# Gallicchio-Lab/openmm_agbnp_plugin

Measured on AMD Instinct MI355X. Metric: AGBNP1 force-eval-limited ns/day (1 fs step), thrombin 1dwc, independent replicas, higher is better.
Workload: dtype f64

## Files before the change

openmm_agbnp_plugin_amd/csrc/decompose_kernels.hip:

```cpp
#define AGBNP_GROUP_TU
#include "pair_bodies.h"

namespace agbnp {

__device__ __forceinline__ void decompose_atoms(const PairArgs& P, int version, int i, double* __restrict__ per_atom) {
  if (i >= P.n) return;
  const size_t n = (size_t)P.n;
  const int h = P.a2h[i];
  if (h >= 0) hbm_add(&per_atom[i], P.gam_cav[h] * (P.sv_large[h] - P.sv_vdw[h]));
  if (version != 1) return;
  const double b = P.born[i], q = P.charge[i], bh = b + kHBRadius;
  hbm_add(&per_atom[n + i], P.alpha[i] / (bh * bh * bh));
  hbm_add(&per_atom[2 * n + i], kDielFactor * q * q / b);
}

template <bool kCut>
__device__ __forceinline__ void decompose_tile(const PairArgs& P, int tile, double* __restrict__ plane) {
  __shared__ double2 s_xy[128], s_zq[128], s_bb[128];
  __shared__ double2 s_ixy[64], s_izq[64], s_ibc[64];
  __shared__ double s_red[4][2][64];
  __shared__ double s_box[2][6];
  const int n = P.n, nb = (n + 63) >> 6;
  if (tile >= nb * (nb + 1) / 2) return;
  int I = (int)(0.5 * ((double)(2 * nb + 1) - sqrt((double)(2 * nb + 1) * (double)(2 * nb + 1) - 8.0 * (double)tile)));
  I = max(0, min(I, nb - 1));
  while (I > 0 && I * nb - I * (I - 1) / 2 > tile) I--;
  while (I + 1 < nb && (I + 1) * nb - (I + 1) * I / 2 <= tile) I++;
  const int J = I + (tile - (I * nb - I * (I - 1) / 2));
  const int lane = threadIdx.x & 63, wave = threadIdx.x >> 6;
  const bool diag = I == J;
  if (wave < 2) {
    const int a = 64 * (wave == 0 ? J : I) + lane;
    const bool va = a < n;
    const int ac = va ? a : n - 1;
    const double4 pa = P.aposq[ac];
    const double br = P.born[ac], inv_br = 1.0 / br;
    const double qa = va ? pa.w : 0.0;
    if (wave == 0) {
      s_xy[lane] = s_xy[lane + 64] = make_double2(pa.x, pa.y);
      s_zq[lane] = s_zq[lane + 64] = make_double2(pa.z, qa);
      s_bb[lane] = s_bb[lane + 64] = make_double2(br, inv_br);
    } else {
      s_ixy[lane] = make_double2(pa.x, pa.y);
      s_izq[lane] = make_double2(pa.z, qa);
      s_ibc[lane] = make_double2(br, (-0.25 * 1.4426950408889634074) * inv_br);
    }
    if (kCut && !diag) {
      double lo[3] = {pa.x, pa.y, pa.z}, hi[3] = {pa.x, pa.y, pa.z};
      for (int off = 32; off > 0; off >>= 1)
        for (int d = 0; d < 3; d++) {
          lo[d] = fmin(lo[d], __shfl_xor(lo[d], off, 64));
          hi[d] = fmax(hi[d], __shfl_xor(hi[d], off, 64));
        }
      if (lane == 0)
        for (int d = 0; d < 3; d++) s_box[wave][d] = lo[d], s_box[wave][3 + d] = hi[d];
    }
  }
  __syncthreads();
  if (kCut && !diag) {
    if (box_gap2(&s_box[0][0], 0, 1) >= P.gb_cut2) return;
  }
  const int nsteps = diag ? 8 : 16;
  const int start = (diag ? 1 : 0) + nsteps * wave;
  const double2 ixy = s_ixy[lane], izq = s_izq[lane], ibc = s_ibc[lane];
  const double xi = ixy.x, yi = ixy.y, zi = izq.x, qi = izq.y, bi = ibc.x, ci = ibc.y;
  const int masked_step = diag ? 32 - start : -1;
  const double qlast = lane >= 32 ? 0.0 : qi;
  const int base = (lane + start) & 63;
  const double2* __restrict__ jxy = s_xy + base;
  const double2* __restrict__ jzq = s_zq + base;
  const double2* __restrict__ jbb = s_bb + base;
  double ei = 0.0, ej = 0.0;
#pragma unroll 8
  for (int k = 0; k < nsteps; k++) {
    const double2 xy = jxy[k], zq = jzq[k], bj = jbb[k];
    const double dx = xy.x - xi, dy = xy.y - yi, dz = zq.x - zi;
    const double d2 = fma(dz, dz, fma(dy, dy, dx * dx));
    double qq = (k == masked_step ? qlast : qi) * zq.y;
// ... 40 lines not shown
```

openmm_agbnp_plugin_amd/csrc/device_math.h:

```cpp
#pragma once
#include <hip/hip_runtime.h>

namespace agbnp {

__device__ __forceinline__ double exp2_nonpositive(double y) {
  y = fmax(y, -96.0);
  const double kShift = 6755399441055744.0;
  const double t = y + kShift;
  const double f = y - (t - kShift);
  double p = 0x1.e6063f7217bc6p-28;
  p = fma(p, f, 0x1.b675bca4eeebbp-24);
  p = fma(p, f, 0x1.62bfd47773353p-20);
  p = fma(p, f, 0x1.ffcb54062e698p-17);
  p = fma(p, f, 0x1.430913096fd9fp-13);
  p = fma(p, f, 0x1.5d87fe9d7a584p-10);
  p = fma(p, f, 0x1.3b2ab6fba1ddap-7);
  p = fma(p, f, 0x1.c6b08d703ce49p-5);
  p = fma(p, f, 0x1.ebfbdff82c598p-3);
  p = fma(p, f, 0x1.62e42fefa3a19p-1);
  p = fma(p, f, 1.0);
  const int n = __double2loint(t);
  return __hiloint2double(__double2hiint(p) + (n << 20), __double2loint(p));
}

__device__ __forceinline__ double rsqrt_pos(double u) {
  const double y0 = __builtin_amdgcn_rsq(u);
  const double e = fma(-(u * y0), y0, 1.0);
  return fma(y0 * e, fma(0.375, e, 0.5), y0);
}

__device__ __forceinline__ double exp_nonpositive(double x) { return exp2_nonpositive(x * 1.4426950408889634074); }

constexpr double kQGrad = 17179869184.0;
constexpr double kQVol = 4503599627370496.0;
constexpr double kQBorn = 17592186044416.0;
constexpr double kQSum = 1099511627776.0;
constexpr double kQEnergy = 68719476736.0;
__device__ __forceinline__ double quantize(double v, double scale, bool det) { return det ? rint(v * scale) * (1.0 / scale) : v; }

__device__ __forceinline__ double pow_three_halves(double q) { return (q * q) * rsqrt_pos(q); }

}
```

openmm_agbnp_plugin_amd/csrc/pair_bodies.h:

```cpp
#pragma once
#include <hip/hip_runtime.h>

#include <algorithm>

#include "agbnp_common.h"
#include "device_math.h"
#include "pair_kernels.h"
#include "group_args.h"
#include "prep_role.h"

namespace agbnp {

#ifdef AGBNP_PAIR_STAMPS
constexpr int kPairLogSlots = 4096;
__device__ unsigned long long g_pair_log[3][kPairLogSlots][12];
#define PAIR_STAMP(kern, idx)                                                                                        \
  do {                                                                                                               \
    if (threadIdx.x == 0 && blockIdx.x < kPairLogSlots) g_pair_log[kern][blockIdx.x][idx] = wall_clock64();          \
  } while (0)
#define PAIR_STAMP_WAIT(kern, idx, what)                                                                            \
  do {                                                                                                               \
    asm volatile("s_waitcnt " what ::: "memory");                                                                    \
    PAIR_STAMP(kern, idx);                                                                                           \
  } while (0)
// ... 48 lines not shown
  c.c3 = hi.y - lo.y;
  return c;
}
__device__ __forceinline__ double spline_value(const double2* __restrict__ tab, int base, double d) {
  const SplineCubic c = spline_cubic(tab, base, d);
  return fma(fma(fma(c.c3, c.t, c.c2), c.t, c.c1), c.t, c.c0);
}
__device__ __forceinline__ void spline_value_deriv(const double2* __restrict__ tab, int base, double d, double& val, double& der) {
  const SplineCubic c = spline_cubic(tab, base, d);
  val = fma(fma(fma(c.c3, c.t, c.c2), c.t, c.c1), c.t, c.c0);
  der = fma(fma(3.0 * c.c3, c.t, 2.0 * c.c2), c.t, c.c1) * ((kI4Nodes - 1) / kI4MaxA);
}

struct LutBatch {
  double2 v[4];
};
__device__ __forceinline__ LutBatch lut_fetch(const double2* __restrict__ lut, int lut_entries, int base) {
  LutBatch b;
#pragma unroll
  for (int r = 0; r < 4; r++) b.v[r] = lut[min(base + (int)threadIdx.x + 256 * r, lut_entries - 1)];
  return b;
}
__device__ __forceinline__ void lut_store(double2* __restrict__ s_lut, const LutBatch& b, int lut_entries, int base) {
#pragma unroll
  for (int r = 0; r < 4; r++) {
    const int t = base + (int)threadIdx.x + 256 * r;
    if (t < lut_entries) s_lut[t] = b.v[r];
  }
}
__device__ __forceinline__ void lut_copy_rest(double2* __restrict__ s_lut, const double2* __restrict__ lut, int lut_entries) {
  for (int base = 1024; base < lut_entries; base += 1024) lut_store(s_lut, lut_fetch(lut, lut_entries, base), lut_entries, base);
}

__device__ void neighbor_tile(const PairArgs& P, int tile, bool write_ref = false) {
  __shared__ double s_x[128], s_y[128], s_z[128];
  __shared__ unsigned short s_bits[4][64];
  const int t = threadIdx.x;
  const int nhb = (P.nh + 63) >> 6;
  int I = (int)(0.5 * ((double)(2 * nhb + 1) - sqrt((double)(2 * nhb + 1) * (double)(2 * nhb + 1) - 8.0 * (double)tile)));
  I = max(0, min(I, nhb - 1));
  while (I > 0 && I * nhb - I * (I - 1) / 2 > tile) I--;
  while (I + 1 < nhb && (I + 1) * nhb - (I + 1) * I / 2 <= tile) I++;
  if (nhb == 0 || tile >= nhb * (nhb + 1) / 2) return;
  const int J = I + (tile - (I * nhb - I * (I - 1) / 2));
  if (t < 128) {
    const int h = 64 * (t < 64 ? I : J) + (t & 63);
    const Pos3 r = heavy_position(P, h < P.nh ? h : P.nh - 1);
    s_x[t] = r.x;
    s_y[t] = r.y;
    s_z[t] = r.z;
  }
  __syncthreads();
  if (write_ref && I == J && t < 64 && 64 * I + t < P.nh) {
    P.mask_ref[3 * (64 * I + t)] = s_x[t];
    P.mask_ref[3 * (64 * I + t) + 1] = s_y[t];
    P.mask_ref[3 * (64 * I + t) + 2] = s_z[t];
  }
  const int li = t & 63, jq = t >> 6, hi = 64 * I + li;
  const double xi = s_x[li], yi = s_y[li], zi = s_z[li];
  const int j0 = 16 * jq;
  unsigned hits = 0;
#pragma unroll
  for (int jj = 0; jj < 16; jj++) {
    const int lj = j0 + jj, hj = 64 * J + lj;
    const double dx = s_x[64 + lj] - xi, dy = s_y[64 + lj] - yi, dz = s_z[64 + lj] - zi;
    if (hj < P.nh && hj > hi && dx * dx + dy * dy + dz * dz < P.mask_rcut2) hits |= 1u << jj;
  }
  s_bits[jq][li] = (unsigned short)hits;
  __syncthreads();
// ... 586 lines not shown

__device__ __forceinline__ double box_gap2(const double* box, int I, int J) {
  double gap2 = 0.0;
  for (int d = 0; d < 3; d++) {
    const double g = fmax(0.0, fmax(box[6 * J + d] - box[6 * I + 3 + d], box[6 * I + d] - box[6 * J + 3 + d]));
    gap2 += g * g;
  }
  return gap2;
}
__device__ __forceinline__ double strip_gap2(const PairArgs& P, int I0, int J) {
  return fmin(fmin(1e300, box_gap2(P.abox, I0, J)), box_gap2(P.abox, I0 + 1, J));
}
__device__ __forceinline__ void gb_energy_put(double e, double* s_e, int lane, int wave) {
  e = wave_sum(e);
  if (lane == 0) s_e[wave] = e;
}
__device__ __forceinline__ void gb_energy_store(const double* s_e, double* out) {
  if (threadIdx.x == 0) out[0] = 2.0 * kDielFactor * ((s_e[0] + s_e[1]) + (s_e[2] + s_e[3]));
}
__device__ __forceinline__ int wave_max_hi_to_lane63(int m) {
  m = max(m, __builtin_amdgcn_update_dpp(m, m, 0x111, 0xf, 0xf, false));
  m = max(m, __builtin_amdgcn_update_dpp(m, m, 0x112, 0xf, 0xf, false));
  m = max(m, __builtin_amdgcn_update_dpp(m, m, 0x114, 0xf, 0xf, false));
  m = max(m, __builtin_amdgcn_update_dpp(m, m, 0x118, 0xf, 0xf, false));
  m = max(m, __builtin_amdgcn_update_dpp(m, m, 0x142, 0xa, 0xf, false));
  m = max(m, __builtin_amdgcn_update_dpp(m, m, 0x143, 0xc, 0xf, false));
  return m;
}

constexpr double kGbFarFactor = 4.0 * 60.0 * 0.69314718055994530942;
template <bool kCut, bool kFar, bool kEnergy = false>
__device__ __forceinline__ void gb_strip(int n, int I0, int J, const double4* __restrict__ aposq, const double* __restrict__ born_part,
                                         const double* __restrict__ inv_rvdw, double* __restrict__ gb_rows, double* __restrict__ egb_out,
                                         const PairArgs& P, char* s_area, double* s_e, int* s_bmax) {
  double2* const s_xy = reinterpret_cast<double2*>(s_area);
  double2* const s_zq = s_xy + 128;
  double2* const s_bb = s_zq + 128;
  double2* const s_i = s_bb + 128;
  const int lane = threadIdx.x & 63, wave = threadIdx.x >> 6;
  if (kCut) {
    if (strip_gap2(P, I0, J) >= P.gb_cut2) {
      if (threadIdx.x == 0) egb_out[0] = 0.0;
      return;
    }
  }
  const double far_gap2 = kFar ? strip_gap2(P, I0, J) : 0.0;
  PAIR_STAMP_WHERE(1, make_tile_item(I0, J, kTileStripFlag));
  const int ysa = P.a2s[min(64 * I0 + lane, n - 1)], ysc = P.a2s[min(64 * I0 + 64 + lane, n - 1)], ysj = P.a2s[min(64 * J + lane, n - 1)];
  double beta_a = 0.0, beta_c = 0.0, beta_j = 0.0;
  if (!kEnergy && P.rows_on && wave == 3) {
    const int ka = min(64 * I0 + lane, n - 1), kc = min(64 * I0 + 64 + lane, n - 1), kj = min(64 * J + lane, n - 1);
    const double ra = inv_rvdw[ka], rc = inv_rvdw[kc], rj = inv_rvdw[kj], pa = born_part[ka], pc = born_part[kc], pj = born_part[kj];
    beta_a = bw_beta(born_radius(ra, pa));
    beta_c = bw_beta(born_radius(rc, pc));
    beta_j = bw_beta(born_radius(rj, pj));
  }
  if (wave < 3) {
    const int a = 64 * (wave == 0 ? J : I0 + wave - 1) + lane;
    const bool va = a < n;
    const int ac = va ? a : n - 1;
    const double4 pa = aposq[ac];
    const BornRadius bra = born_radius(inv_rvdw[ac], born_part[ac]);
    const double qa = va ? pa.w : 0.0;
    if (wave == 0) {
      s_xy[lane] = s_xy[lane + 64] = make_double2(pa.x, pa.y);
      s_zq[lane] = s_zq[lane + 64] = make_double2(pa.z, qa);
      s_bb[lane] = s_bb[lane + 64] = make_double2(bra.br, bra.inv_br);
    } else {
      double2* r = s_i + (wave - 1) * 192;
      r[lane] = make_double2(pa.x, pa.y);
      r[64 + lane] = make_double2(pa.z, qa);
      r[128 + lane] = make_double2(bra.br, (-0.25 * 1.4426950408889634074) * bra.inv_br);
    }
    if (kFar) {
      const int m = wave_max_hi_to_lane63(__double2hiint(bra.br));
      if (lane == 63) s_bmax[wave] = m + 1;
    }
  }
  __syncthreads();
  PAIR_STAMP(1, 1);
  __builtin_amdgcn_s_setprio(0);
  const int start = 16 * wave;
  const double2 axy = s_i[lane], azq = s_i[64 + lane], abc = s_i[128 + lane];
  const double2 cxy = s_i[192 + lane], czq = s_i[256 + lane], cbc = s_i[320 + lane];
  const int base = (lane + start) & 63;
  const double2* __restrict__ jxy = s_xy + base;
  const double2* __restrict__ jzq = s_zq + base;
  const double2* __restrict__ jbb = s_bb + base;
  double fxa = 0, fya = 0, fza = 0, ya = 0, fxc = 0, fyc = 0, fzc = 0, yc = 0, fxj = 0, fyj = 0, fzj = 0, yj = 0, e = 0;
  bool far = false;
  if (kFar) {
    const double bj = __hiloint2double(s_bmax[0], 0), bi = __hiloint2double(max(s_bmax[1], s_bmax[2]), 0);
    far = __builtin_amdgcn_readfirstlane(far_gap2 > kGbFarFactor * bj * bi ? 1 : 0) != 0;
  }
  if (kFar && far) {
#pragma unroll 4
    for (int k = 0; k < 16; k++) {
      const double2 xy = jxy[k], zq = jzq[k];
      const double dxa = xy.x - axy.x, dya = xy.y - axy.y, dza = zq.x - azq.x;
      const double d2a = fma(dza, dza, fma(dya, dya, dxa * dxa));
      const double fa = rsqrt_pos(d2a);
      const double s1a = (azq.y * zq.y) * fa;
      const double mwa = s1a * (fa * fa);
      const double dxc = xy.x - cxy.x, dyc = xy.y - cxy.y, dzc = zq.x - czq.x;
      const double d2c = fma(dzc, dzc, fma(dyc, dyc, dxc * dxc));
      const double fc = rsqrt_pos(d2c);
      const double s1c = (czq.y * zq.y) * fc;
      const double mwc = s1c * (fc * fc);
      e += s1a + s1c;
      fxa = fma(dxa, mwa, fxa);
      fya = fma(dya, mwa, fya);
      fza = fma(dza, mwa, fza);
      fxc = fma(dxc, mwc, fxc);
      fyc = fma(dyc, mwc, fyc);
      fzc = fma(dzc, mwc, fzc);
      fxj = rot1(fma(-dxa, mwa, fma(-dxc, mwc, fxj)));
      fyj = rot1(fma(-dya, mwa, fma(-dyc, mwc, fyj)));
      fzj = rot1(fma(-dza, mwa, fma(-dzc, mwc, fzj)));
    }
  } else
#pragma unroll 4
  for (int k = 0; k < 16; k++) {
    const double2 xy = jxy[k], zq = jzq[k], bj = jbb[k];
    const double dxa = xy.x - axy.x, dya = xy.y - axy.y, dza = zq.x - azq.x;
    const double d2a = fma(dza, dza, fma(dya, dya, dxa * dxa));
    double qqa = azq.y * zq.y;
    if (kCut) qqa = d2a < P.gb_cut2 ? qqa : 0.0;
    const GbPairTerms<double> ta = gb_pair_terms(d2a, abc.x * bj.x, abc.y * bj.y, qqa);
    const double mwa = ta.mw, yta = ta.ybb * ta.ets3;
    const double dxc = xy.x - cxy.x, dyc = xy.y - cxy.y, dzc = zq.x - czq.x;
    const double d2c = fma(dzc, dzc, fma(dyc, dyc, dxc * dxc));
    double qqc = czq.y * zq.y;
    if (kCut) qqc = d2c < P.gb_cut2 ? qqc : 0.0;
    const GbPairTerms<double> tc = gb_pair_terms(d2c, cbc.x * bj.x, cbc.y * bj.y, qqc);
    const double mwc = tc.mw, ytc = tc.ybb * tc.ets3;
    e += ta.s1 + tc.s1;
    fxa = fma(dxa, mwa, fxa);
    fya = fma(dya, mwa, fya);
    fza = fma(dza, mwa, fza);
    ya += yta;
    fxc = fma(dxc, mwc, fxc);
    fyc = fma(dyc, mwc, fyc);
    fzc = fma(dzc, mwc, fzc);
    yc += ytc;
    fxj = rot1(fma(-dxa, mwa, fma(-dxc, mwc, fxj)));
    fyj = rot1(fma(-dya, mwa, fma(-dyc, mwc, fyj)));
    fzj = rot1(fma(-dza, mwa, fma(-dzc, mwc, fzj)));
    yj = rot1(yj + (yta + ytc));
  }
  const double kf = -2.0 * kDielFactor;
  __builtin_amdgcn_s_setprio(3);
  __syncthreads();
  PAIR_STAMP(1, 2);
  StripSums& S = *reinterpret_cast<StripSums*>(s_area);
  const int jslot = (lane + start + 16) & 63;
  if (kEnergy) {
    gb_energy_put(e, s_e, lane, wave);
    __syncthreads();
    return gb_energy_store(s_e, egb_out);
  }
  S.red[wave][0][lane] = kf * fxa;
  S.red[wave][1][lane] = kf * fya;
  S.red[wave][2][lane] = kf * fza;
  S.red[wave][3][lane] = ya;
  S.red[wave][4][lane] = kf * fxc;
  S.red[wave][5][lane] = kf * fyc;
  S.red[wave][6][lane] = kf * fzc;
  S.red[wave][7][lane] = yc;
  S.red[wave][8][jslot] = kf * fxj;
  S.red[wave][9][jslot] = kf * fyj;
  S.red[wave][10][jslot] = kf * fzj;
  S.red[wave][11][jslot] = yj;
  gb_energy_put(e, s_e, lane, wave);
  __syncthreads();
  double* __restrict__ row = gb_rows + (size_t)wave * n;
  auto fold = [&](int r) { return (S.red[0][r][lane] + S.red[1][r][lane]) + (S.red[2][r][lane] + S.red[3][r][lane]); };
  const int ia = 64 * I0 + lane, ic = ia + 64, j = 64 * J + lane;
  const bool det = P.det != 0;
  const double qs = wave == 3 ? kQSum : kQGrad;
  if (kFar && far && wave == 3) {
  } else if (P.rows_on && wave == 3) {
    if (ia < n) hbm_add(&P.bw[ia], beta_a * fold(3));
    if (ic < n) hbm_add(&P.bw[ic], beta_c * fold(7));
    if (j < n) hbm_add(&P.bw[j], beta_j * fold(11));
  } else {
    if (ia < n) hbm_add(wave == 3 ? &P.ys[ysa] : &row[ia], quantize(fold(wave), qs, det));
    if (ic < n) hbm_add(wave == 3 ? &P.ys[ysc] : &row[ic], quantize(fold(4 + wave), qs, det));
    if (j < n) hbm_add(wave == 3 ? &P.ys[ysj] : &row[j], quantize(fold(8 + wave), qs, det));
  }
  gb_energy_store(s_e, egb_out);
  PAIR_STAMP(1, 3);
}

typedef float v2f __attribute__((ext_vector_type(2)));
__device__ __forceinline__ float rot1f(float v) {
  return __int_as_float(__builtin_amdgcn_update_dpp(0, __float_as_int(v), 0x134, 0xf, 0xf, true));
}
template <bool kCut>
__device__ __forceinline__ void gb_strip_f32(int n, int I0, int J, const double4* __restrict__ aposq, const double* __restrict__ born_part,
                                             const double* __restrict__ inv_rvdw, double* __restrict__ gb_rows, double* __restrict__ egb_out,
                                             const PairArgs& P, char* s_area, double* s_e) {
  float4* const s_jr = reinterpret_cast<float4*>(s_area);
  float2* const s_jb = reinterpret_cast<float2*>(s_jr + 128);
  float4* const s_ir = reinterpret_cast<float4*>(s_jb + 128);
  float2* const s_ib = reinterpret_cast<float2*>(s_ir + 128);
  static_assert(sizeof(StripSums) >= 128 * 16 + 128 * 8 + 128 * 16 + 128 * 8, "single-precision records fit the area of the sums");
  const int lane = threadIdx.x & 63, wave = threadIdx.x >> 6;
  if (kCut) {
    if (strip_gap2(P, I0, J) >= P.gb_cut2) {
      if (threadIdx.x == 0) egb_out[0] = 0.0;
      return;
    }
  }
  const int ysa = P.a2s[min(64 * I0 + lane, n - 1)], ysc = P.a2s[min(64 * I0 + 64 + lane, n - 1)], ysj = P.a2s[min(64 * J + lane, n - 1)];
  const double4 origin = aposq[min(64 * J, n - 1)];
  if (wave < 3) {
    const int a = 64 * (wave == 0 ? J : I0 + wave - 1) + lane;
// ... 64 lines not shown
  S.red[wave][8][jslot] = kf * (double)fxj;
  S.red[wave][9][jslot] = kf * (double)fyj;
  S.red[wave][10][jslot] = kf * (double)fzj;
  S.red[wave][11][jslot] = (double)yj;
  gb_energy_put((double)e2.x + (double)e2.y, s_e, lane, wave);
  __syncthreads();
  double* __restrict__ row = gb_rows + (size_t)wave * n;
  auto fold = [&](int r) { return (S.red[0][r][lane] + S.red[1][r][lane]) + (S.red[2][r][lane] + S.red[3][r][lane]); };
  const int ia = 64 * I0 + lane, ic = ia + 64, j = 64 * J + lane;
  const bool det = P.det != 0;
  const double qs = wave == 3 ? kQSum : kQGrad;
  if (ia < n) hbm_add(wave == 3 ? &P.ys[ysa] : &row[ia], quantize(fold(wave), qs, det));
  if (ic < n) hbm_add(wave == 3 ? &P.ys[ysc] : &row[ic], quantize(fold(4 + wave), qs, det));
  if (j < n) hbm_add(wave == 3 ? &P.ys[ysj] : &row[j], quantize(fold(8 + wave), qs, det));
  gb_energy_store(s_e, egb_out);
}

template <bool kCut, bool kSingle, bool kFar, bool kMasks = false, bool kEnergy = false>
AGBNP_KERNEL AGBNP_BOUNDS(256) void k_gb_tiles(int n, const int* __restrict__ items, const double4* __restrict__ aposq,
                                                  const double* __restrict__ born_part, const double* __restrict__ inv_rvdw,
                                                  const double* __restrict__ alpha, double* __restrict__ born,
                                                  double* __restrict__ born_fp, double* __restrict__ brw,
                                                  double* __restrict__ e_atom, double* __restrict__ gb_rows,
                                                  double* __restrict__ egb_part, PairArgs P AGBNP_WG_PARAM) {
  if (kMasks && (int)AGBNP_WG > P.gb_items_count) {
    if (((P.estatus[kStatOrderStale] & 2) | P.estatus[kStatMaskAging]) == 0) return;
    return neighbor_tile(P, (int)AGBNP_WG - 1 - P.gb_items_count, true);
  }
  __shared__ __align__(16) char s_area[sizeof(StripSums)];
  static_assert(sizeof(StripSums) >= sizeof(TileSums) && sizeof(TileSums) >= kRoleScratchBytes, "the packing workgroup borrows the tile area");
  static_assert(sizeof(StripSums) >= sizeof(double2) * (3 * 128 + 6 * 64), "strip records fit the area of the sums");
  __shared__ double s_e[4];
  __shared__ int s_bmax[4];
  if (AGBNP_WG == 0) {
    PAIR_STAMP(1, 0);
    rebase_for_parity(P, 0);
    packing_role<true>(P, s_area, (int)sizeof(StripSums));
    PAIR_STAMP(1, 3);
    return;
  }
  static_assert(sizeof(TileSums) >= sizeof(double2) * (3 * 128 + 3 * 64), "records fit the area of the sums");
  double2* const s_xy = reinterpret_cast<double2*>(s_area);
  double2* const s_zq = s_xy + 128;
  double2* const s_bb = s_zq + 128;
  double2* const s_ixy = s_bb + 128;
  double2* const s_izq = s_ixy + 64;
  double2* const s_ibc = s_izq + 64;
  const int lane = threadIdx.x & 63, wave = threadIdx.x >> 6;
  __builtin_amdgcn_s_setprio(3);
  const int item = items[AGBNP_WG - 1];
  const int I = tile_I(item), J = tile_J(item);
  PAIR_STAMP(1, 0);
  if (item & kTileStripFlag) {
    if (kSingle) return gb_strip_f32<kCut>(n, I, J, aposq, born_part, inv_rvdw, gb_rows, egb_part + (AGBNP_WG - 1), P, s_area, s_e);
    return gb_strip<kCut, kFar, kEnergy>(n, I, J, aposq, born_part, inv_rvdw, gb_rows, egb_part + (AGBNP_WG - 1), P, s_area, s_e, s_bmax);
  }
  const bool diag = I == J;
  if (kCut && !diag) {
    if (box_gap2(P.abox, I, J) >= P.gb_cut2) {
      if (threadIdx.x == 0) egb_part[AGBNP_WG - 1] = 0.0;
      return;
    }
  }
  PAIR_STAMP_WHERE(1, item);
  const int ysi = P.a2s[min(64 * I + lane, n - 1)], ysj = P.a2s[min(64 * J + lane, n - 1)];
  double beta_i = 0.0, beta_j = 0.0;
  if (!kEnergy && P.rows_on && wave == 3) {
    const int ki = min(64 * I + lane, n - 1), kj = min(64 * J + lane, n - 1);
    const double ri = inv_rvdw[ki], rj = inv_rvdw[kj], pi = born_part[ki], pj = born_part[kj];
    beta_i = bw_beta(born_radius(ri, pi));
    beta_j = bw_beta(born_radius(rj, pj));
  }
  if (wave < 2) {
    const int a = 64 * (wave == 0 ? J : I) + lane;
    const bool va = a < n;
    const int ac = va ? a : n - 1;
    const double4 pa = aposq[ac];
    const BornRadius bra = born_radius(inv_rvdw[ac], born_part[ac]);
    const double qa = va ? pa.w : 0.0;
    if (wave == 0) {
      s_xy[lane] = s_xy[lane + 64] = make_double2(pa.x, pa.y);
      s_zq[lane] = s_zq[lane + 64] = make_double2(pa.z, qa);
      s_bb[lane] = s_bb[lane + 64] = make_double2(bra.br, bra.inv_br);
    } else {
      s_ixy[lane] = make_double2(pa.x, pa.y);
      s_izq[lane] = make_double2(pa.z, qa);
      s_ibc[lane] = make_double2(bra.br, (-0.25 * 1.4426950408889634074) * bra.inv_br);
      if (diag && va) {
        const double brw_a = publish_atom(a, bra, pa.w, alpha, born, born_fp, e_atom, brw, P.bw, !kEnergy && P.rows_on);
        P.srec[ysi] = make_double4(bra.br, bra.fp, brw_a, pa.w);
      }
    }
  }
  __syncthreads();
  PAIR_STAMP(1, 1);
  __builtin_amdgcn_s_setprio(0);
  const int nsteps = diag ? 8 : 16;
  const int start = (diag ? 1 : 0) + nsteps * wave;
  const double2 ixy = s_ixy[lane], izq = s_izq[lane], ibc = s_ibc[lane];
  const double xi = ixy.x, yi_ = ixy.y, zi = izq.x, qi = izq.y, bi = ibc.x, ci = ibc.y;
  const int masked_step = diag ? 32 - start : -1;
  const double qlast = lane >= 32 ? 0.0 : qi;
  const int base = (lane + start) & 63;
  const double2* __restrict__ jxy = s_xy + base;
  const double2* __restrict__ jzq = s_zq + base;
  const double2* __restrict__ jbb = s_bb + base;
  double fxi = 0, fyi = 0, fzi = 0, yi = 0, fxj = 0, fyj = 0, fzj = 0, yj_acc = 0, e = 0;
#pragma unroll 8
  for (int k = 0; k < nsteps; k++) {
    const double2 xy = jxy[k], zq = jzq[k], bj = jbb[k];
    const double dx = xy.x - xi, dy = xy.y - yi_, dz = zq.x - zi;
    const double d2 = fma(dz, dz, fma(dy, dy, dx * dx));
    double qq = (k == masked_step ? qlast : qi) * zq.y;
    if (kCut) qq = d2 < P.gb_cut2 ? qq : 0.0;
    const GbPairTerms<double> t = gb_pair_terms(d2, bi * bj.x, ci * bj.y, qq);
    const double mw = t.mw;
    e += t.s1;
    fxi = fma(dx, mw, fxi);
    fyi = fma(dy, mw, fyi);
    fzi = fma(dz, mw, fzi);
    fxj = fma(-dx, mw, fxj);
    fyj = fma(-dy, mw, fyj);
    fzj = fma(-dz, mw, fzj);
    const double yt = t.ybb * t.ets3;
    yi += yt;
    yj_acc += yt;
    fxj = rot1(fxj);
    fyj = rot1(fyj);
    fzj = rot1(fzj);
    yj_acc = rot1(yj_acc);
  }
  const double kf = -2.0 * kDielFactor;
  __builtin_amdgcn_s_setprio(3);
  __syncthreads();
  PAIR_STAMP(1, 2);
  TileSums& s_sums = *reinterpret_cast<TileSums*>(s_area);
  if (kEnergy) {
    gb_energy_put(e, s_e, lane, wave);
    __syncthreads();
    return gb_energy_store(s_e, egb_part + (AGBNP_WG - 1));
  }
  {
    const double vi4[4] = {kf * fxi, kf * fyi, kf * fzi, yi}, vj4[4] = {kf * fxj, kf * fyj, kf * fzj, yj_acc};
    tile_sums_store(s_sums, wave, lane, (lane + start + nsteps) & 63, vi4, vj4);
  }
  gb_energy_put(e, s_e, lane, wave);
  __syncthreads();
  double* __restrict__ row = gb_rows + (size_t)wave * n;
  const int i = 64 * I + lane, j = 64 * J + lane;
  const bool det = P.det != 0;
  const double qs = wave == 3 ? kQSum : kQGrad;
  if (P.rows_on && wave == 3) {
    if (i < n) hbm_add(&P.bw[i], beta_i * tile_sums_fold(s_sums, 3, lane));
    if (j < n) hbm_add(&P.bw[j], beta_j * tile_sums_fold(s_sums, 7, lane));
  } else {
    if (i < n) hbm_add(wave == 3 ? &P.ys[ysi] : &row[i], quantize(tile_sums_fold(s_sums, wave, lane), qs, det));
    if (j < n) hbm_add(wave == 3 ? &P.ys[ysj] : &row[j], quantize(tile_sums_fold(s_sums, 4 + wave, lane), qs, det));
  }
  gb_energy_store(s_e, egb_part + (AGBNP_WG - 1));
  PAIR_STAMP(1, 3);
}

template <int KIND, bool SINGLE = false, bool MASKS = false, bool DEVPAR = false>
AGBNP_KERNEL AGBNP_BOUNDS(64 * row_waves(KIND), KIND == kGbRows ? 4 : 6) void k_rows(PairArgs P, double* __restrict__ energy_out, double* __restrict__ components, int role_arg AGBNP_WG_PARAM) {
  extern __shared__ double2 s_dyn[];

  int blk = AGBNP_WG;
  if (MASKS && KIND == kBornRows && blk >= role_arg) {
    if (threadIdx.x >= 256) return;
    if (DEVPAR) rebase_for_parity(P, 0);
    if (((P.estatus[kStatOrderStale] & 2) | P.estatus[kStatMaskAging]) == 0) return;
    return neighbor_tile(P, blk - role_arg, true);
  }
  if (KIND == kChainRows) {
    if (blk < 2 && threadIdx.x >= 256) return;
    if (blk == 0) return energy_role<DEVPAR>(P, 1, energy_out, components, reinterpret_cast<char*>(s_dyn));
    if (blk == 1) return dealing_role(P, reinterpret_cast<char*>(s_dyn), role_arg);
    blk -= 2;
  }
  if (KIND == kGbRows) {
    if (blk == 0) {
      static_assert(kGbRowWaves >= 4, "the bookkeeping role is written for 256 lanes");
      if (threadIdx.x >= 256) return;
      PAIR_STAMP(1, 0);
      rebase_for_parity(P, 0);
      packing_role<false>(P, reinterpret_cast<char*>(s_dyn), role_arg);
      PAIR_STAMP(1, 3);
// ... 72 lines not shown
```

openmm_agbnp_plugin_amd/csrc/row_kernels.h:

```cpp
#pragma once
#include <hip/hip_runtime.h>

#include "agbnp_common.h"
#include "device_math.h"
#include "pair_kernels.h"

#ifndef PAIR_STAMP
#define PAIR_STAMP(kern, idx)
#define PAIR_STAMP_WAIT(kern, idx, what)
#define PAIR_STAMP_WHERE(kern, item)
#endif
#ifndef PAIR_STAMP_HW
#define PAIR_STAMP_HW(kern)
#endif
#ifndef ROWS_LOG_COUNTS
#define ROWS_LOG_COUNTS(kern, todo, nsteps)
#endif

namespace agbnp {

__device__ __forceinline__ void hbm_add(double* p, double v) {
  __hip_atomic_fetch_add(p, v, __ATOMIC_RELAXED, __HIP_MEMORY_SCOPE_AGENT);
}

// ... 4 lines not shown

struct BornRadius {
  double br, inv_br, fp;
};
__device__ __forceinline__ BornRadius born_radius(double inv_rvdw, double qsum) {
  const double beta = inv_rvdw - (1. / (4. * kPi)) * qsum;
  const double amin = 1. / kI4MaxA, a2 = 1. / (kI4MaxA * kI4MaxA);
  BornRadius r;
  if (beta < 0.0) {
    r.inv_br = amin;
    r.fp = 0.0;
  } else {
    r.inv_br = sqrt(a2 + beta * beta);
    r.fp = beta / r.inv_br;
  }
  r.br = 1. / r.inv_br;
  return r;
}
__device__ __forceinline__ double bw_beta(const BornRadius& r) { return -(1. / (4. * kPi)) * kDielFactor * r.br * r.fp; }
__device__ __forceinline__ double bw_alpha(const BornRadius& r, double brw, double q) { return brw - (1. / (4. * kPi)) * kDielFactor * (q * q) * r.fp; }

__device__ __forceinline__ double publish_atom(int a, const BornRadius& r, double q, const double* alpha, double* born, double* born_fp,
                                               double* e_atom, double* brw, double* bw, bool add_bw) {
  const double bh = r.br + kHBRadius, bh3 = bh * bh * bh, al = alpha[a];
  const double brw_a = -(1. / (4. * kPi)) * 3. * al * r.br * r.br * r.fp / (bh3 * bh);
  born[a] = r.br;
  born_fp[a] = r.fp;
  e_atom[a] = al / bh3 + kDielFactor * q * q * r.inv_br;
  brw[a] = brw_a;
  if (add_bw) hbm_add(&bw[a], bw_alpha(r, brw_a, q));
  return brw_a;
}
template <class real>
struct GbPairTerms {
  real s1, mw, ybb, ets3;
};
__device__ __forceinline__ double gb_exp2(double y) { return exp2_nonpositive(y); }
__device__ __forceinline__ float gb_exp2(float y) { return __builtin_amdgcn_exp2f(y); }
__device__ __forceinline__ double gb_rsqrt(double u) { return rsqrt_pos(u); }
__device__ __forceinline__ float gb_rsqrt(float u) { return __builtin_amdgcn_rsqf(u); }
template <class real>
__device__ __forceinline__ GbPairTerms<real> gb_pair_terms(real d2, real bb, real c, real qq) {
  const real et = gb_exp2(d2 * c), fgb = gb_rsqrt(fma(bb, et, d2));
  GbPairTerms<real> t;
  t.s1 = qq * fgb;
  const real s3 = t.s1 * (fgb * fgb);
  t.mw = fma((real)-0.25, et, (real)1) * s3, t.ybb = fma((real)0.25, d2, bb), t.ets3 = et * s3;
  return t;
}

constexpr int kRowIntervals = kI4Nodes - 1;

__device__ __forceinline__ int uniform(int v) { return __builtin_amdgcn_readfirstlane(v); }
__device__ __forceinline__ double uniform(double v) {
  return __hiloint2double(__builtin_amdgcn_readfirstlane(__double2hiint(v)), __builtin_amdgcn_readfirstlane(__double2loint(v)));
}
template <int kCtrl>
__device__ __forceinline__ double dpp_move(double v) {
  const int lo = __builtin_amdgcn_update_dpp(0, __double2loint(v), kCtrl, 0xf, 0xf, true);
  const int hi = __builtin_amdgcn_update_dpp(0, __double2hiint(v), kCtrl, 0xf, 0xf, true);
  return __hiloint2double(hi, lo);
}
__device__ __forceinline__ double lane_xor1(double v) { return dpp_move<0xB1>(v); }
__device__ __forceinline__ double lane_xor2(double v) { return dpp_move<0x4E>(v); }
__device__ __forceinline__ double lane_xor4(double v) { return dpp_move<0x1B>(dpp_move<0x141>(v)); }
__device__ __forceinline__ double lane_xor8(double v) { return dpp_move<0x128>(v); }

enum RowKind { kBornRows = 0, kChainRows = 1, kGbRows = 2 };
struct RowAtoms {
  double x[kRowGroup], y[kRowGroup], z[kRowGroup];
  int self[kRowGroup];
  int rows;
};

template <int KIND>
__device__ __forceinline__ RowAtoms row_atoms(const PairArgs& P, int group) {
  RowAtoms A;
  const int nrows = KIND == kChainRows ? P.nh : P.n;
  A.rows = min(kRowGroup, nrows - kRowGroup * group);
  const double4* __restrict__ pos = KIND == kChainRows ? static_cast<const double4*>(P.hrow) : static_cast<const double4*>(P.aposq);
// ... 300 lines not shown
      e2 = list[min(first + 64 * (k + 2) + lane, stride - 1)];
      const int b = (int)row_entry_index(e);
      const int tent = (int)row_entry_type(e) * kRowIntervals;
      const double w = (KIND == kChainRows ? wb : wb * rb.w) * kPerNode;
      const double range2 = 64 * k + lane < todo ? P.range2 : -1.0;
#pragma unroll
      for (int r = 0; r < R; r++) {
        const double dx = rb.x - A.x[r], dy = rb.y - A.y[r], dz = rb.z - A.z[r];
        const double d2 = fma(dz, dz, fma(dy, dy, dx * dx));
        if (d2 < range2 && b != A.self[r]) {
          const double rinv = rsqrt_pos(d2);
          const double u = fmin((d2 * rinv) * kPerNode, kRowIntervals - 0x1p-49);
          const int ent = slice_at[r] + tent + (int)u;
          const double t = __builtin_amdgcn_fract(u);
          const double2 ca = s_tab[ent], cb = s_tab[ent + tab];
          const double b2 = fma(cb.y, t, cb.x), b1 = fma(b2, t, ca.y);
          const double val = fma(b1, t, ca.x), der = fma(fma(cb.y, t, b2), t, b1);
          acc[4 * r] = fma(w, val, acc[4 * r]);
          const double g = w * der * rinv;
          acc[4 * r + 1] = fma(dx, g, acc[4 * r + 1]);
          acc[4 * r + 2] = fma(dy, g, acc[4 * r + 2]);
          acc[4 * r + 3] = fma(dz, g, acc[4 * r + 3]);
        }
      }
    }
  } else {
    const double4* __restrict__ rec = static_cast<const double4*>(P.aposq);
    double qa[R], ba[R], ca_[R];
    BornRadius bra[R];
#pragma unroll
    for (int r = 0; r < R; r++) {
      bra[r] = born_radius(row_rv[r], row_bp[r]);
      qa[r] = uniform(r < A.rows ? row_q[r] : 0.0);
      ba[r] = uniform(bra[r].br);
      ca_[r] = uniform((-0.25 * 1.4426950408889634074) * bra[r].inv_br);
      beta_r[r] = bw_beta(bra[r]);
    }
    if (active && slice == 0 && part == 0 && lane < A.rows) {
      BornRadius br = bra[0];
      double qv = row_q[0];
#pragma unroll
      for (int r = 1; r < R; r++) {
        if (lane == r) br = bra[r], qv = row_q[r];
      }
      publish_atom(R * group + lane, br, qv, P.alpha, P.born, P.born_fp, P.e_atom, P.brw, P.bw, true);
    }
    double4 r1 = rec[row_entry_index(e1)];
    double p1 = P.born_part[row_entry_index(e1)], v1 = P.inv_rvdw[row_entry_index(e1)];
    PAIR_STAMP(kRowStamp<KIND>, 8);
    PAIR_STAMP_WAIT(kRowStamp<KIND>, 1, "vmcnt(0)");
    ROWS_LOG_COUNTS(kRowStamp<KIND>, todo, nsteps);
    if (P.single) {
      float ox[R], oy[R], oz[R], qf[R], bf[R], cf[R], accf[4 * R];
#pragma unroll
      for (int r = 0; r < R; r++) {
        ox[r] = (float)(A.x[r] - A.x[0]), oy[r] = (float)(A.y[r] - A.y[0]), oz[r] = (float)(A.z[r] - A.z[0]);
        qf[r] = (float)qa[r], bf[r] = (float)ba[r], cf[r] = (float)ca_[r];
      }
#pragma unroll
      for (int q = 0; q < 4 * R; q++) accf[q] = 0.0f;
      float esumf = 0.0f;
      for (int k = 0; k < nsteps; k++) {
        const unsigned e = e1;
        const double4 rb = r1;
        const BornRadius bb_ = born_radius(v1, p1);
        e1 = e2;
        r1 = rec[row_entry_index(e1)];
        p1 = P.born_part[row_entry_index(e1)], v1 = P.inv_rvdw[row_entry_index(e1)];
        e2 = list[min(first + 64 * (k + 2) + lane, stride - 1)];
        const int b = (int)row_entry_index(e);
        const float cut2 = 64 * k + lane < todo ? (float)P.gb_cut2 : -1.0f;
        const float nx = (float)(rb.x - A.x[0]), ny = (float)(rb.y - A.y[0]), nz = (float)(rb.z - A.z[0]);
        const float qb = (float)rb.w, bj = (float)bb_.br, ibj = (float)bb_.inv_br;
#pragma unroll
        for (int r = 0; r < R; r++) {
          const float dx = nx - ox[r], dy = ny - oy[r], dz = nz - oz[r];
          const float d2 = fmaf(dz, dz, fmaf(dy, dy, dx * dx));
          if (d2 < cut2 && b != A.self[r]) {
            const GbPairTerms<float> t = gb_pair_terms(d2, bf[r] * bj, cf[r] * ibj, qf[r] * qb);
            esumf += t.s1;
            accf[4 * r] = fmaf(t.ybb, t.ets3, accf[4 * r]);
            accf[4 * r + 1] = fmaf(dx, t.mw, accf[4 * r + 1]);
            accf[4 * r + 2] = fmaf(dy, t.mw, accf[4 * r + 2]);
            accf[4 * r + 3] = fmaf(dz, t.mw, accf[4 * r + 3]);
          }
        }
      }
#pragma unroll
      for (int q = 0; q < 4 * R; q++) acc[q] = (double)accf[q];
      esum = (double)esumf;
    } else
    for (int k = 0; k < nsteps; k++) {
      const unsigned e = e1;
      const double4 rb = r1;
      const BornRadius bb_ = born_radius(v1, p1);
      e1 = e2;
      r1 = rec[row_entry_index(e1)];
      p1 = P.born_part[row_entry_index(e1)], v1 = P.inv_rvdw[row_entry_index(e1)];
      e2 = list[min(first + 64 * (k + 2) + lane, stride - 1)];
      const int b = (int)row_entry_index(e);
      const double cut2 = 64 * k + lane < todo ? P.gb_cut2 : -1.0;
#pragma unroll
      for (int r = 0; r < R; r++) {
        const double dx = rb.x - A.x[r], dy = rb.y - A.y[r], dz = rb.z - A.z[r];
        const double d2 = fma(dz, dz, fma(dy, dy, dx * dx));
        if (d2 < cut2 && b != A.self[r]) {
          const double bb = ba[r] * bb_.br;
          const double et = exp2_nonpositive(d2 * (ca_[r] * bb_.inv_br));
          const double fgb = rsqrt_pos(fma(bb, et, d2));
          const double s1 = (qa[r] * rb.w) * fgb;
          esum += s1;
          const double s3 = s1 * (fgb * fgb);
          const double mw = fma(-0.25, et, 1.0) * s3;
          acc[4 * r] = fma(fma(0.25, d2, bb), et * s3, acc[4 * r]);
          acc[4 * r + 1] = fma(dx, mw, acc[4 * r + 1]);
          acc[4 * r + 2] = fma(dy, mw, acc[4 * r + 2]);
          acc[4 * r + 3] = fma(dz, mw, acc[4 * r + 3]);
        }
      }
    }
    esum = wave_sum(esum);
    if (lane == 0 && item < P.egb_parts) P.egb_part[item] = kDielFactor * esum;
  }
  PAIR_STAMP(kRowStamp<KIND>, 2);
  if (nsteps == 0) return;
  const bool u0 = lane & 1, u1 = lane & 2, u2 = lane & 4, u3 = lane & 8;
#pragma unroll
  for (int q = 0; q < 8; q++) acc[q] = (u0 ? acc[q + 8] : acc[q]) + lane_xor1(u0 ? acc[q] : acc[q + 8]);
#pragma unroll
  for (int q = 0; q < 4; q++) acc[q] = (u1 ? acc[q + 4] : acc[q]) + lane_xor2(u1 ? acc[q] : acc[q + 4]);
#pragma unroll
  for (int q = 0; q < 2; q++) acc[q] = (u2 ? acc[q + 2] : acc[q]) + lane_xor4(u2 ? acc[q] : acc[q + 2]);
  double total = (u3 ? acc[1] : acc[0]) + lane_xor8(u3 ? acc[0] : acc[1]);
  total += __shfl_xor(total, 16, 64);
  total += __shfl_xor(total, 32, 64);
  const int q = ((lane & 1) << 3) | ((lane & 2) << 1) | ((lane & 4) >> 1) | ((lane & 8) >> 3);
  const int r = q >> 2, c = q & 3;
  if (lane < 16 && r < A.rows) {
    const int row = R * group + r;
    if (KIND == kGbRows) {
      double beta = 0.0;
#pragma unroll
      for (int rr = 0; rr < R; rr++) beta = rr == r ? beta_r[rr] : beta;
      if (c == 0)
        hbm_add(&P.bw[row], beta * total);
      else
        hbm_add(P.gb_fx + (size_t)(c - 1) * P.n + row, (-2.0 * kDielFactor) * total);
// ... 11 lines not shown
```

Before: 884.5.

## Fold -1/4 into exp polynomial and reuse Born beta via LDS

Scales the exp2 polynomial coefficients by -1/4 and pre-multiplies the Born product by -4. This removes a separate fma when forming mw and yt, and simplifies yt to s1 - d2*mw. The gb_strip and tile kernels now compute the Born-weight beta once in the loader waves and pass it through a new LDS array, instead of having wave 3 reload inv_rvdw and born_part and recompute born_radius. In exchange it adds LDS per workgroup and changes floating-point rounding, which matters for the deterministic quantization.

```diff
diff --git a/openmm_agbnp_plugin_amd/csrc/decompose_kernels.hip b/openmm_agbnp_plugin_amd/csrc/decompose_kernels.hip
--- a/openmm_agbnp_plugin_amd/csrc/decompose_kernels.hip
+++ b/openmm_agbnp_plugin_amd/csrc/decompose_kernels.hip
@@ -43,7 +43,7 @@
     } else {
       s_ixy[lane] = make_double2(pa.x, pa.y);
       s_izq[lane] = make_double2(pa.z, qa);
-      s_ibc[lane] = make_double2(br, (-0.25 * 1.4426950408889634074) * inv_br);
+      s_ibc[lane] = make_double2(-4.0 * br, (-0.25 * 1.4426950408889634074) * inv_br);
     }
     if (kCut && !diag) {
       double lo[3] = {pa.x, pa.y, pa.z}, hi[3] = {pa.x, pa.y, pa.z};
diff --git a/openmm_agbnp_plugin_amd/csrc/device_math.h b/openmm_agbnp_plugin_amd/csrc/device_math.h
--- a/openmm_agbnp_plugin_amd/csrc/device_math.h
+++ b/openmm_agbnp_plugin_amd/csrc/device_math.h
@@ -23,6 +23,26 @@
   return __hiloint2double(__double2hiint(p) + (n << 20), __double2loint(p));
 }
 
+__device__ __forceinline__ double exp2_nonpositive_negquarter(double y) {
+  y = fmax(y, -96.0);
+  const double kShift = 6755399441055744.0;
+  const double t = y + kShift;
+  const double f = y - (t - kShift);
+  double p = -0x1.e6063f7217bc6p-30;
+  p = fma(p, f, -0x1.b675bca4eeebbp-26);
+  p = fma(p, f, -0x1.62bfd47773353p-22);
+  p = fma(p, f, -0x1.ffcb54062e698p-19);
+  p = fma(p, f, -0x1.430913096fd9fp-15);
+  p = fma(p, f, -0x1.5d87fe9d7a584p-12);
+  p = fma(p, f, -0x1.3b2ab6fba1ddap-9);
+  p = fma(p, f, -0x1.c6b08d703ce49p-7);
+  p = fma(p, f, -0x1.ebfbdff82c598p-5);
+  p = fma(p, f, -0x1.62e42fefa3a19p-3);
+  p = fma(p, f, -0.25);
+  const int n = __double2loint(t);
+  return __hiloint2double(__double2hiint(p) + (n << 20), __double2loint(p));
+}
+
 __device__ __forceinline__ double rsqrt_pos(double u) {
   const double y0 = __builtin_amdgcn_rsq(u);
   const double e = fma(-(u * y0), y0, 1.0);
diff --git a/openmm_agbnp_plugin_amd/csrc/pair_bodies.h b/openmm_agbnp_plugin_amd/csrc/pair_bodies.h
--- a/openmm_agbnp_plugin_amd/csrc/pair_bodies.h
+++ b/openmm_agbnp_plugin_amd/csrc/pair_bodies.h
@@ -104,9 +104,11 @@
   for (int base = 1024; base < lut_entries; base += 1024) lut_store(s_lut, lut_fetch(lut, lut_entries, base), lut_entries, base);
 }
 
+constexpr int kNeighborTileLds = 3 * 128 * (int)sizeof(double) + 4 * 64 * (int)sizeof(unsigned short);
 __device__ void neighbor_tile(const PairArgs& P, int tile, bool write_ref = false) {
   __shared__ double s_x[128], s_y[128], s_z[128];
   __shared__ unsigned short s_bits[4][64];
+  static_assert(sizeof(s_x) + sizeof(s_y) + sizeof(s_z) + sizeof(s_bits) == kNeighborTileLds, "kNeighborTileLds names these arrays");
   const int t = threadIdx.x;
   const int nhb = (P.nh + 63) >> 6;
   int I = (int)(0.5 * ((double)(2 * nhb + 1) - sqrt((double)(2 * nhb + 1) * (double)(2 * nhb + 1) - 8.0 * (double)tile)));
@@ -759,7 +761,7 @@
 template <bool kCut, bool kFar, bool kEnergy = false>
 __device__ __forceinline__ void gb_strip(int n, int I0, int J, const double4* __restrict__ aposq, const double* __restrict__ born_part,
                                          const double* __restrict__ inv_rvdw, double* __restrict__ gb_rows, double* __restrict__ egb_out,
-                                         const PairArgs& P, char* s_area, double* s_e, int* s_bmax) {
+                                         const PairArgs& P, char* s_area, double* s_e, int* s_bmax, double (*s_beta)[64]) {
   double2* const s_xy = reinterpret_cast<double2*>(s_area);
   double2* const s_zq = s_xy + 128;
   double2* const s_bb = s_zq + 128;
@@ -774,14 +776,7 @@
   const double far_gap2 = kFar ? strip_gap2(P, I0, J) : 0.0;
   PAIR_STAMP_WHERE(1, make_tile_item(I0, J, kTileStripFlag));
   const int ysa = P.a2s[min(64 * I0 + lane, n - 1)], ysc = P.a2s[min(64 * I0 + 64 + lane, n - 1)], ysj = P.a2s[min(64 * J + lane, n - 1)];
-  double beta_a = 0.0, beta_c = 0.0, beta_j = 0.0;
-  if (!kEnergy && P.rows_on && wave == 3) {
-    const int ka = min(64 * I0 + lane, n - 1), kc = min(64 * I0 + 64 + lane, n - 1), kj = min(64 * J + lane, n - 1);
-    const double ra = inv_rvdw[ka], rc = inv_rvdw[kc], rj = inv_rvdw[kj], pa = born_part[ka], pc = born_part[kc], pj = born_part[kj];
-    beta_a = bw_beta(born_radius(ra, pa));
-    beta_c = bw_beta(born_radius(rc, pc));
-    beta_j = bw_beta(born_radius(rj, pj));
-  }
+  const bool bw_shares = !kEnergy && P.rows_on;
   if (wave < 3) {
     const int a = 64 * (wave == 0 ? J : I0 + wave - 1) + lane;
     const bool va = a < n;
@@ -797,8 +792,9 @@
       double2* r = s_i + (wave - 1) * 192;
       r[lane] = make_double2(pa.x, pa.y);
       r[64 + lane] = make_double2(pa.z, qa);
-      r[128 + lane] = make_double2(bra.br, (-0.25 * 1.4426950408889634074) * bra.inv_br);
-    }
+      r[128 + lane] = make_double2(-4.0 * bra.br, (-0.25 * 1.4426950408889634074) * bra.inv_br);
+    }
+    if (bw_shares) s_beta[wave][lane] = bw_beta(bra);
     if (kFar) {
       const int m = wave_max_hi_to_lane63(__double2hiint(bra.br));
       if (lane == 63) s_bmax[wave] = m + 1;
@@ -854,13 +850,13 @@
     double qqa = azq.y * zq.y;
     if (kCut) qqa = d2a < P.gb_cut2 ? qqa : 0.0;
     const GbPairTerms<double> ta = gb_pair_terms(d2a, abc.x * bj.x, abc.y * bj.y, qqa);
-    const double mwa = ta.mw, yta = ta.ybb * ta.ets3;
+    const double mwa = ta.mw, yta = ta.yt;
     const double dxc = xy.x - cxy.x, dyc = xy.y - cxy.y, dzc = zq.x - czq.x;
     const double d2c = fma(dzc, dzc, fma(dyc, dyc, dxc * dxc));
     double qqc = czq.y * zq.y;
     if (kCut) qqc = d2c < P.gb_cut2 ? qqc : 0.0;
     const GbPairTerms<double> tc = gb_pair_terms(d2c, cbc.x * bj.x, cbc.y * bj.y, qqc);
-    const double mwc = tc.mw, ytc = tc.ybb * tc.ets3;
+    const double mwc = tc.mw, ytc = tc.yt;
     e += ta.s1 + tc.s1;
     fxa = fma(dxa, mwa, fxa);
     fya = fma(dya, mwa, fya);
@@ -907,9 +903,9 @@
   const double qs = wave == 3 ? kQSum : kQGrad;
   if (kFar && far && wave == 3) {
   } else if (P.rows_on && wave == 3) {
-    if (ia < n) hbm_add(&P.bw[ia], beta_a * fold(3));
-    if (ic < n) hbm_add(&P.bw[ic], beta_c * fold(7));
-    if (j < n) hbm_add(&P.bw[j], beta_j * fold(11));
+    if (ia < n) hbm_add(&P.bw[ia], s_beta[1][lane] * fold(3));
+    if (ic < n) hbm_add(&P.bw[ic], s_beta[2][lane] * fold(7));
+    if (j < n) hbm_add(&P.bw[j], s_beta[0][lane] * fold(11));
   } else {
     if (ia < n) hbm_add(wave == 3 ? &P.ys[ysa] : &row[ia], quantize(fold(wave), qs, det));
     if (ic < n) hbm_add(wave == 3 ? &P.ys[ysc] : &row[ic], quantize(fold(4 + wave), qs, det));
@@ -1040,6 +1036,9 @@
   static_assert(sizeof(StripSums) >= sizeof(double2) * (3 * 128 + 6 * 64), "strip records fit the area of the sums");
   __shared__ double s_e[4];
   __shared__ int s_bmax[4];
+  __shared__ double s_beta[3][64];
+  static_assert(4 * (sizeof(StripSums) + sizeof(s_beta) + sizeof(s_e) + sizeof(s_bmax) + (kMasks ? kNeighborTileLds : 0)) <= 160 * 1024,
+                "four workgroups of the launch share a CU's 160 KB of LDS (26.1 KB each, 29.7 KB with the mask tiles)");
   if (AGBNP_WG == 0) {
     PAIR_STAMP(1, 0);
     rebase_for_parity(P, 0);
@@ -1061,7 +1060,7 @@
   PAIR_STAMP(1, 0);
   if (item & kTileStripFlag) {
     if (kSingle) return gb_strip_f32<kCut>(n, I, J, aposq, born_part, inv_rvdw, gb_rows, egb_part + (AGBNP_WG - 1), P, s_area, s_e);
-    return gb_strip<kCut, kFar, kEnergy>(n, I, J, aposq, born_part, inv_rvdw, gb_rows, egb_part + (AGBNP_WG - 1), P, s_area, s_e, s_bmax);
+    return gb_strip<kCut, kFar, kEnergy>(n, I, J, aposq, born_part, inv_rvdw, gb_rows, egb_part + (AGBNP_WG - 1), P, s_area, s_e, s_bmax, s_beta);
   }
   const bool diag = I == J;
   if (kCut && !diag) {
@@ -1072,13 +1071,7 @@
   }
   PAIR_STAMP_WHERE(1, item);
   const int ysi = P.a2s[min(64 * I + lane, n - 1)], ysj = P.a2s[min(64 * J + lane, n - 1)];
-  double beta_i = 0.0, beta_j = 0.0;
-  if (!kEnergy && P.rows_on && wave == 3) {
-    const int ki = min(64 * I + lane, n - 1), kj = min(64 * J + lane, n - 1);
-    const double ri = inv_rvdw[ki], rj = inv_rvdw[kj], pi = born_part[ki], pj = born_part[kj];
-    beta_i = bw_beta(born_radius(ri, pi));
-    beta_j = bw_beta(born_radius(rj, pj));
-  }
+  const bool bw_shares = !kEnergy && P.rows_on;
   if (wave < 2) {
     const int a = 64 * (wave == 0 ? J : I) + lane;
     const bool va = a < n;
@@ -1086,6 +1079,7 @@
     const double4 pa = aposq[ac];
     const BornRadius bra = born_radius(inv_rvdw[ac], born_part[ac]);
     const double qa = va ? pa.w : 0.0;
+    if (bw_shares) s_beta[wave][lane] = bw_beta(bra);
     if (wave == 0) {
       s_xy[lane] = s_xy[lane + 64] = make_double2(pa.x, pa.y);
       s_zq[lane] = s_zq[lane + 64] = make_double2(pa.z, qa);
@@ -1093,7 +1087,7 @@
     } else {
       s_ixy[lane] = make_double2(pa.x, pa.y);
       s_izq[lane] = make_double2(pa.z, qa);
-      s_ibc[lane] = make_double2(bra.br, (-0.25 * 1.4426950408889634074) * bra.inv_br);
+      s_ibc[lane] = make_double2(-4.0 * bra.br, (-0.25 * 1.4426950408889634074) * bra.inv_br);
       if (diag && va) {
         const double brw_a = publish_atom(a, bra, pa.w, alpha, born, born_fp, e_atom, brw, P.bw, !kEnergy && P.rows_on);
         P.srec[ysi] = make_double4(bra.br, bra.fp, brw_a, pa.w);
@@ -1130,7 +1124,7 @@
     fxj = fma(-dx, mw, fxj);
     fyj = fma(-dy, mw, fyj);
     fzj = fma(-dz, mw, fzj);
-    const double yt = t.ybb * t.ets3;
+    const double yt = t.yt;
     yi += yt;
     yj_acc += yt;
     fxj = rot1(fxj);
@@ -1159,8 +1153,8 @@
   const bool det = P.det != 0;
   const double qs = wave == 3 ? kQSum : kQGrad;
   if (P.rows_on && wave == 3) {
-    if (i < n) hbm_add(&P.bw[i], beta_i * tile_sums_fold(s_sums, 3, lane));
-    if (j < n) hbm_add(&P.bw[j], beta_j * tile_sums_fold(s_sums, 7, lane));
+    if (i < n) hbm_add(&P.bw[i], s_beta[1][lane] * tile_sums_fold(s_sums, 3, lane));
+    if (j < n) hbm_add(&P.bw[j], s_beta[0][lane] * tile_sums_fold(s_sums, 7, lane));
   } else {
     if (i < n) hbm_add(wave == 3 ? &P.ys[ysi] : &row[i], quantize(tile_sums_fold(s_sums, wave, lane), qs, det));
     if (j < n) hbm_add(wave == 3 ? &P.ys[ysj] : &row[j], quantize(tile_sums_fold(s_sums, 4 + wave, lane), qs, det));
diff --git a/openmm_agbnp_plugin_amd/csrc/row_kernels.h b/openmm_agbnp_plugin_amd/csrc/row_kernels.h
--- a/openmm_agbnp_plugin_amd/csrc/row_kernels.h
+++ b/openmm_agbnp_plugin_amd/csrc/row_kernels.h
@@ -60,20 +60,29 @@
   return brw_a;
 }
 template <class real>
-struct GbPairTerms {
-  real s1, mw, ybb, ets3;
+struct GbPairTerms;
+template <>
+struct GbPairTerms<double> {
+  double s1, mw, yt;
 };
-__device__ __forceinline__ double gb_exp2(double y) { return exp2_nonpositive(y); }
-__device__ __forceinline__ float gb_exp2(float y) { return __builtin_amdgcn_exp2f(y); }
-__device__ __forceinline__ double gb_rsqrt(double u) { return rsqrt_pos(u); }
-__device__ __forceinline__ float gb_rsqrt(float u) { return __builtin_amdgcn_rsqf(u); }
-template <class real>
-__device__ __forceinline__ GbPairTerms<real> gb_pair_terms(real d2, real bb, real c, real qq) {
-  const real et = gb_exp2(d2 * c), fgb = gb_rsqrt(fma(bb, et, d2));
-  GbPairTerms<real> t;
+__device__ __forceinline__ GbPairTerms<double> gb_pair_terms(double d2, double bb4, double c, double qq) {
+  const double et4 = exp2_nonpositive_negquarter(d2 * c), fgb = rsqrt_pos(fma(bb4, et4, d2));
+  GbPairTerms<double> t;
   t.s1 = qq * fgb;
-  const real s3 = t.s1 * (fgb * fgb);
-  t.mw = fma((real)-0.25, et, (real)1) * s3, t.ybb = fma((real)0.25, d2, bb), t.ets3 = et * s3;
+  const double s3 = t.s1 * (fgb * fgb);
+  t.mw = fma(et4, s3, s3), t.yt = fma(-d2, t.mw, t.s1);
+  return t;
+}
+template <>
+struct GbPairTerms<float> {
+  float s1, mw, ybb, ets3;
+};
+__device__ __forceinline__ GbPairTerms<float> gb_pair_terms(float d2, float bb, float c, float qq) {
+  const float et = __builtin_amdgcn_exp2f(d2 * c), fgb = __builtin_amdgcn_rsqf(fmaf(bb, et, d2));
+  GbPairTerms<float> t;
+  t.s1 = qq * fgb;
+  const float s3 = t.s1 * (fgb * fgb);
+  t.mw = fmaf(-0.25f, et, 1.0f) * s3, t.ybb = fmaf(0.25f, d2, bb), t.ets3 = et * s3;
   return t;
 }
 
@@ -440,7 +449,7 @@
     for (int r = 0; r < R; r++) {
       bra[r] = born_radius(row_rv[r], row_bp[r]);
       qa[r] = uniform(r < A.rows ? row_q[r] : 0.0);
-      ba[r] = uniform(bra[r].br);
+      ba[r] = __hiloint2double((uniform(__double2hiint(bra[r].br)) ^ (int)0x80000000) + (2 << 20), uniform(__double2loint(bra[r].br)));
       ca_[r] = uniform((-0.25 * 1.4426950408889634074) * bra[r].inv_br);
       beta_r[r] = bw_beta(bra[r]);
     }
@@ -463,7 +472,7 @@
 #pragma unroll
       for (int r = 0; r < R; r++) {
         ox[r] = (float)(A.x[r] - A.x[0]), oy[r] = (float)(A.y[r] - A.y[0]), oz[r] = (float)(A.z[r] - A.z[0]);
-        qf[r] = (float)qa[r], bf[r] = (float)ba[r], cf[r] = (float)ca_[r];
+        qf[r] = (float)qa[r], bf[r] = (float)(-0.25 * ba[r]), cf[r] = (float)ca_[r];
       }
 #pragma unroll
       for (int q = 0; q < 4 * R; q++) accf[q] = 0.0f;
@@ -513,14 +522,13 @@
         const double dx = rb.x - A.x[r], dy = rb.y - A.y[r], dz = rb.z - A.z[r];
         const double d2 = fma(dz, dz, fma(dy, dy, dx * dx));
         if (d2 < cut2 && b != A.self[r]) {
-          const double bb = ba[r] * bb_.br;
-          const double et = exp2_nonpositive(d2 * (ca_[r] * bb_.inv_br));
-          const double fgb = rsqrt_pos(fma(bb, et, d2));
+          const double et4 = exp2_nonpositive_negquarter(d2 * (ca_[r] * bb_.inv_br));
+          const double fgb = rsqrt_pos(fma(ba[r] * bb_.br, et4, d2));
           const double s1 = (qa[r] * rb.w) * fgb;
           esum += s1;
           const double s3 = s1 * (fgb * fgb);
-          const double mw = fma(-0.25, et, 1.0) * s3;
-          acc[4 * r] = fma(fma(0.25, d2, bb), et * s3, acc[4 * r]);
+          const double mw = fma(et4, s3, s3);
+          acc[4 * r] += fma(-d2, mw, s1);
           acc[4 * r + 1] = fma(dx, mw, acc[4 * r + 1]);
           acc[4 * r + 2] = fma(dy, mw, acc[4 * r + 2]);
           acc[4 * r + 3] = fma(dz, mw, acc[4 * r + 3]);
```

Result: no change. 888.5, median of 6 (+0.5%).
